# databendlabs/databend

Hardware: AMD Instinct MI355X
Metric: rows/s TPC-H Q1 hash-agg (higher is better)
Workload: dtype i64/i128 decimal

## Files before the change

### databend_amd/csrc/k_fagg.hip

```cpp
#include "fagg_device.h"
#include "runtime.h"

#include <dirent.h>
#include <dlfcn.h>
#include <errno.h>
#include <sys/stat.h>
#include <fcntl.h>
#include <signal.h>
#include <spawn.h>
#include <sys/wait.h>
#include <unistd.h>

#include <atomic>
#include <chrono>
#include <deque>
#include <map>
#include <mutex>
#include <string>

#include <stdlib.h>
#include <string.h>
#include <time.h>

using namespace dbhip;
// ... 495 lines not shown
    if (keys[k].type != L.key_type[k]) { set_error("dbhip_groupby_add_block_program: key %d has type %d, table expects %d", k, keys[k].type, L.key_type[k]); return DBHIP_ERR_INVALID; }
    if (keys[k].validity && !L.key_nullable[k]) { set_error("dbhip_groupby_add_block_program: key %d carries validity but was declared NOT NULL", k); return DBHIP_ERR_INVALID; }
    GbCol& c = A.key[k];
    c.data = keys[k].data; c.validity = keys[k].validity; c.voff = keys[k].validity_offset; c.buffers = keys[k].buffers;
    c.type = keys[k].type; c.is_scalar = keys[k].is_scalar;
    A.key_type[k] = L.key_type[k]; A.key_off[k] = L.key_off[k]; A.key_words[k] = L.key_words[k];
    A.key_has_valid[k] = keys[k].validity != nullptr;
  }
  *out_general = general; *out_nwords = nwords; *out_may_raise = may_raise;
  return DBHIP_OK;
}


static int32_t fa_launch(const FaArgs& A, int slots, bool general, int nwords, int grid, size_t lds, hipStream_t s) {
  bool jit_pending = false;
  hipFunction_t jf = jit_kernel(A, slots, general, nwords, (t_jit_only && !t_jit_may_compile) ? JIT_LOOKUP : JIT_BACKGROUND, &jit_pending);
  if (!jf && t_jit_only) {
    t_jit_pending = jit_pending;
    if (jit_pending) ++g_fa_pending_refusals;
    set_error("dbhip_fagg: the specialised kernel of this shape is %s", jit_pending ? "being compiled in the background" : "not available");
    return DBHIP_ERR_UNSUPPORTED;
  }
  if (jf) {
    size_t asz = sizeof(A);
    void* extra[] = {HIP_LAUNCH_PARAM_BUFFER_POINTER, (void*)&A, HIP_LAUNCH_PARAM_BUFFER_SIZE, &asz, HIP_LAUNCH_PARAM_END};
    DBHIP_CHECK(hipModuleLaunchKernel(jf, grid, 1, 1, 256, 1, 1, 0, s, nullptr, extra));
    ++g_fa_jit_launches;
    return DBHIP_OK;
  }
  ++g_fa_interp_launches;
#define FA_LAUNCH(SL, GEN)                                                                                     \
  do {                                                                                                         \
    if (nwords <= 4) hipLaunchKernelGGL((fagg_kernel<SL, GEN, 4>), dim3(grid), dim3(256), lds, s, A);           \
    else hipLaunchKernelGGL((fagg_kernel<SL, GEN, FA_MAXW>), dim3(grid), dim3(256), lds, s, A);                 \
  } while (0)
  bool has_div = false;
  for (int i = 0; i < A.P.n_ins; ++i) has_div |= A.P.ins[i].op == EX_DEC && dec_op_needs_division(A.P.dec[A.P.ins[i].dec_idx]);
  if (has_div && slots == 4) hipLaunchKernelGGL((fagg_kernel<4, true, FA_MAXW, true>), dim3(grid), dim3(256), lds, s, A);
  else if (has_div) hipLaunchKernelGGL((fagg_kernel<8, true, FA_MAXW, true>), dim3(grid), dim3(256), lds, s, A);
  else if (slots == 4 && !general) FA_LAUNCH(4, false);
  else if (slots == 4) FA_LAUNCH(4, true);
  else if (!general) FA_LAUNCH(8, false);
  else FA_LAUNCH(8, true);
#undef FA_LAUNCH
  return DBHIP_OK;
}

namespace {
constexpr int FA_PIPE_WINDOW = 2048;
constexpr int FA_PIPE_BATCH = 512;
constexpr size_t FA_PIPE_COPY_BYTES = 16384;
constexpr size_t FA_PIPE_TABLE_BYTES = 65536;
constexpr int FA_PIPE_RING = 8;
constexpr int64_t FA_PIPE_BIG = 8 << 20;
constexpr int64_t FA_PIPE_BATCH_ROWS = 32 << 20;
struct FaShape { FaArgs A; bool general; int nwords; size_t lds; std::string sig; };
struct FaPending { int shape; FaBlock b; };
struct FaMerge { uint64_t seq; int64_t rows_ub; int64_t blocks; };
struct FaPipe {
  bool on = false, bound = false, slots8 = false;
  bool given_up = false;
  hipStream_t stream = nullptr;
  uint64_t* rows = nullptr;
  int64_t cap_rows = 0;
  uint64_t* ctrl = nullptr;
  uint64_t* status_host = nullptr;
  uint64_t* status_dev = nullptr;
  int64_t rows_ub = 0, window_blocks = 0;
  uint64_t seq = 0;
  std::deque<FaMerge> merges;
  int64_t count_seen = 0;
  std::deque<FaPending> retained;
  int64_t retained_base = 0, submitted = 0;
  std::vector<FaPending> batch;
  int64_t batch_rows = 0;
  std::vector<FaShape> shapes;
  uint64_t* tab_host[FA_PIPE_RING] = {};
  uint64_t* tab_dev[FA_PIPE_RING] = {};
  hipEvent_t tab_ev[FA_PIPE_RING] = {};
  bool tab_used[FA_PIPE_RING] = {};
  int tab_next = 0;
};

__global__ void fa_pipe_seal_kernel(uint64_t* ctrl) {
  if (ctrl[2]) ctrl[1] |= 4;
}
__global__ void fa_pipe_commit_kernel(uint64_t* ctrl, const uint64_t* gctrl, uint64_t* status, uint64_t seq, uint64_t blocks) {
  if (gctrl[1]) ctrl[1] |= 8;
  const bool dirty = (ctrl[1] & 15) != 0;
  if (!dirty) ctrl[3] += blocks;
  ctrl[0] = 0;
  __hip_atomic_store(&status[1], gctrl[0] | (dirty ? (1ULL << 63) : 0ULL), __ATOMIC_RELAXED, __HIP_MEMORY_SCOPE_SYSTEM);
  __hip_atomic_store(&status[0], seq, __ATOMIC_RELEASE, __HIP_MEMORY_SCOPE_SYSTEM);
}

void fa_pipe_poll(FaPipe* pp) {
  uint64_t seq0, cnt, seq1;
  do {
    seq0 = __atomic_load_n(&pp->status_host[0], __ATOMIC_ACQUIRE);
    cnt = __atomic_load_n(&pp->status_host[1], __ATOMIC_ACQUIRE);
    seq1 = __atomic_load_n(&pp->status_host[0], __ATOMIC_ACQUIRE);
  } while (seq0 != seq1);
  const bool dirty = (cnt >> 63) != 0;
  while (!pp->merges.empty() && pp->merges.front().seq <= seq0) {
    if (!dirty) {
      int64_t drop = pp->merges.front().blocks;
      while (drop-- > 0 && !pp->retained.empty()) { pp->retained.pop_front(); ++pp->retained_base; }
    }
    pp->merges.pop_front();
    pp->count_seen = (int64_t)(cnt & ~(1ULL << 63));
  }
}

int32_t fa_pipe_queue_merge(dbhip_groupby* g, FaPipe* pp) {
  if (pp->window_blocks == 0) return DBHIP_OK;
  hipStream_t s = pp->stream;
  fa_pipe_poll(pp);
  int64_t ub = pp->count_seen + pp->rows_ub;
  for (const FaMerge& m : pp->merges) ub += m.rows_ub;
  if (ub * 135 > dbhip_groupby_capacity_internal(g) * 100) {
    const int32_t rc = dbhip_groupby_ensure_room_internal(g, pp->rows_ub, s);
    if (rc) return rc;
    fa_pipe_poll(pp);
    pp->merges.clear();
    pp->count_seen = dbhip_groupby_count_internal(g);
  }
  hipLaunchKernelGGL(fa_pipe_seal_kernel, dim3(1), dim3(1), 0, s, pp->ctrl);
  int32_t rc = dbhip_groupby_merge_rows_deferred_internal(g, pp->rows, pp->rows_ub, &pp->ctrl[0], &pp->ctrl[1], s);
  if (rc) return rc;
  ++pp->seq;
  hipLaunchKernelGGL(fa_pipe_commit_kernel, dim3(1), dim3(1), 0, s, pp->ctrl, dbhip_groupby_ctrl_internal(g), pp->status_dev, pp->seq,
                     (uint64_t)pp->window_blocks);
  DBHIP_LAUNCH_CHECK();
  pp->merges.push_back({pp->seq, pp->rows_ub, pp->window_blocks});
  pp->rows_ub = 0;
  pp->window_blocks = 0;
  return DBHIP_OK;
}

void fa_pipe_args(const FaPipe* pp, const FaPending& P, FaArgs& A) {
  A = pp->shapes[(size_t)P.shape].A;
  for (int c = 0; c < EX_MAX_INPUTS; ++c) { A.P.in_data[c] = P.b.in_data[c]; A.P.in_valid[c] = P.b.in_valid[c]; A.P.in_voff[c] = P.b.in_voff[c]; }
  for (int k = 0; k < FA_KW; ++k) { A.key[k].data = P.b.key_data[k]; A.key[k].validity = P.b.key_valid[k]; A.key[k].voff = P.b.key_voff[k]; }
  A.filter_bits = P.b.filter_bits; A.filter_off = P.b.filter_off; A.n = P.b.n;
}
int32_t fa_pipe_submit(dbhip_groupby* g, FaPipe* pp, const FaPending& P, hipStream_t s) {
  const FaShape& S = pp->shapes[(size_t)P.shape];
  FaArgs A;
  fa_pipe_args(pp, P, A);
  const int64_t nchunks = ceil_div(A.n, 64 * FA_ROWS);
  const int grid = (int)(ceil_div(nchunks, 4) < 512 ? ceil_div(nchunks, 4) : 512);
  const int64_t n_max = (int64_t)grid * FA_MAX_SLOTS;
  if (n_max > pp->cap_rows) { set_error("dbhip_groupby_add_block_program: grid too large for the pipeline's row buffer"); return DBHIP_ERR_INVALID; }
  if (pp->rows_ub + n_max > pp->cap_rows || pp->window_blocks >= FA_PIPE_WINDOW) {
    const int32_t rc = fa_pipe_queue_merge(g, pp);
    if (rc) return rc;
  }
  A.ctrl = pp->ctrl;
  A.partial_rows = pp->rows;
  A.P.err_words = nullptr;
  A.P.err_count = (unsigned long long*)&pp->ctrl[2];
  const int32_t rc = fa_launch(A, (pp->slots8 || pp->count_seen > 4) ? 8 : 4, S.general, S.nwords, grid, S.lds, s);
  if (rc) return rc;
  DBHIP_LAUNCH_CHECK();
  pp->rows_ub += n_max;
  ++pp->window_blocks;
  ++pp->submitted;
  pp->retained.push_back(P);
  return DBHIP_OK;
}

void fa_pack_block(const FaArgs& M, const FaBlock& b, uint64_t* w) {
  w[0] = (uint64_t)b.n;
  for (int ci = 0; ci < M.P.n_inputs; ++ci) {
    const int o = fa_blk_in_off(M, ci);
    w[o] = (uint64_t)b.in_data[ci];
    if (M.P.in_has_valid[ci]) { w[o + 1] = (uint64_t)b.in_valid[ci]; w[o + 2] = (uint64_t)b.in_voff[ci]; }
  }
  for (int q = 0; q < M.nkeys; ++q) {
    const int o = fa_blk_key_off(M, q);
    w[o] = (uint64_t)b.key_data[q];
    if (M.key_has_valid[q]) { w[o + 1] = (uint64_t)b.key_valid[q]; w[o + 2] = (uint64_t)b.key_voff[q]; }
  }
  if (M.has_filter) { const int o = fa_blk_filter_off(M); w[o] = (uint64_t)b.filter_bits; w[o + 1] = (uint64_t)b.filter_off; }
}

int32_t fa_pipe_flush_batch(dbhip_groupby* g, FaPipe* pp) {
  if (pp->batch.empty()) return DBHIP_OK;
  std::vector<FaPending> blocks;
  blocks.swap(pp->batch);
  pp->batch_rows = 0;
  hipStream_t s = pp->stream;
  const int nb = (int)blocks.size();
  const int slots = (pp->slots8 || pp->count_seen > 4) ? 8 : 4;
  const FaShape& S = pp->shapes[(size_t)blocks[0].shape];
  hipFunction_t jf = nb > 1 ? jit_kernel(S.A, slots, S.general, S.nwords, JIT_BACKGROUND, nullptr, true) : nullptr;
  if (!jf) {
    for (const FaPending& P : blocks) { const int32_t rc = fa_pipe_submit(g, pp, P, s); if (rc) return rc; }
    return DBHIP_OK;
  }
  const int64_t rpw = 64 * (int64_t)jit_rows(S.A);
  int64_t max_chunks = 1;
  for (const FaPending& P : blocks) { const int64_t c = ceil_div(P.b.n, rpw); max_chunks = c > max_chunks ? c : max_chunks; }
  int wpb = (int)(ceil_div(max_chunks, 4) < 512 / nb ? ceil_div(max_chunks, 4) : 512 / nb);
  if (wpb < 1) wpb = 1;
  const int grid = wpb * nb;
  const int64_t n_max = (int64_t)grid * FA_MAX_SLOTS;
  if (pp->rows_ub + n_max > pp->cap_rows || pp->window_blocks >= FA_PIPE_WINDOW) {
    const int32_t rc = fa_pipe_queue_merge(g, pp);
    if (rc) return rc;
  }
  const int slot = pp->tab_next;
  pp->tab_next = (pp->tab_next + 1) % FA_PIPE_RING;
  if (pp->tab_used[slot]) DBHIP_CHECK(hipEventSynchronize(pp->tab_ev[slot]));
  uint64_t* T = pp->tab_host[slot];
  const int bw = fa_blk_words(S.A);
  for (int i = 0; i < nb; ++i) fa_pack_block(S.A, blocks[i].b, T + (size_t)i * bw);
  for (size_t at = 0, all = (size_t)nb * bw * 8; at < all; at += FA_PIPE_COPY_BYTES)
    DBHIP_CHECK(hipMemcpyAsync((uint8_t*)pp->tab_dev[slot] + at, (const uint8_t*)T + at, all - at < FA_PIPE_COPY_BYTES ? all - at : FA_PIPE_COPY_BYTES,
                               hipMemcpyHostToDevice, s));
  DBHIP_CHECK(hipEventRecord(pp->tab_ev[slot], s));
  pp->tab_used[slot] = true;
  FaArgs A = S.A;
  A.ctrl = pp->ctrl; A.partial_rows = pp->rows;
  A.P.err_words = nullptr; A.P.err_count = (unsigned long long*)&pp->ctrl[2];
  A.blocks = pp->tab_dev[slot]; A.wgs_per_block = wpb;
  size_t asz = sizeof(A);
  void* extra[] = {HIP_LAUNCH_PARAM_BUFFER_POINTER, (void*)&A, HIP_LAUNCH_PARAM_BUFFER_SIZE, &asz, HIP_LAUNCH_PARAM_END};
  DBHIP_CHECK(hipModuleLaunchKernel(jf, grid, 1, 1, 256, 1, 1, 0, s, nullptr, extra));
  g_fa_jit_launches += 1;
  g_fa_multi_blocks += (uint64_t)nb;
  pp->rows_ub += n_max;
  pp->window_blocks += nb;
  pp->submitted += nb;
  for (const FaPending& P : blocks) pp->retained.push_back(P);
  return DBHIP_OK;
}

int32_t fa_pipe_enqueue(dbhip_groupby* g, FaPipe* pp, const FaPending& P, hipStream_t s) {
  if (P.b.n >= FA_PIPE_BIG || jit_mode() == 0) {
    const int32_t rc = fa_pipe_flush_batch(g, pp);
    return rc ? rc : fa_pipe_submit(g, pp, P, s);
  }
  if (!pp->batch.empty() && pp->batch[0].shape != P.shape) {
    const int32_t rc = fa_pipe_flush_batch(g, pp);
    if (rc) return rc;
  }
  pp->batch.push_back(P);
  pp->batch_rows += P.b.n;
  const int fit = (int)(FA_PIPE_TABLE_BYTES / ((size_t)fa_blk_words(pp->shapes[(size_t)P.shape].A) * 8));
  if ((int)pp->batch.size() >= (FA_PIPE_BATCH < fit ? FA_PIPE_BATCH : fit) || pp->batch_rows >= FA_PIPE_BATCH_ROWS) return fa_pipe_flush_batch(g, pp);
  return DBHIP_OK;
}

void fa_pipe_forget(FaPipe* pp) {
  pp->batch.clear(); pp->batch_rows = 0; pp->shapes.clear();
  pp->retained.clear(); pp->retained_base = 0; pp->submitted = 0; pp->merges.clear(); pp->rows_ub = 0; pp->window_blocks = 0;
}

int32_t fa_pipe_checkpoint(dbhip_groupby* g, FaPipe* pp, int64_t* out_committed, bool may_replay) {
  if (out_committed) *out_committed = 0;
  if (!pp->bound || (pp->submitted == 0 && pp->window_blocks == 0 && pp->batch.empty())) return DBHIP_OK;
  hipStream_t s = pp->stream;
  int32_t rc = fa_pipe_flush_batch(g, pp);
  if (rc) return rc;
  if ((rc = fa_pipe_queue_merge(g, pp))) return rc;
  uint64_t* h = pinned_words(2);
  if (!h) return DBHIP_ERR_HIP;
  DBHIP_CHECK(hipMemcpyAsync(h, pp->ctrl, 32, hipMemcpyDeviceToHost, s));
  DBHIP_CHECK(hipMemcpyAsync(h + 4, dbhip_groupby_ctrl_internal(g), 8, hipMemcpyDeviceToHost, s));
  DBHIP_CHECK(hipStreamSynchronize(s));
  const uint64_t flags = h[1], errs = h[2];
  const int64_t committed = (int64_t)h[3];
  dbhip_groupby_set_count_internal(g, (int64_t)h[4]);
  pp->merges.clear();
  pp->count_seen = (int64_t)h[4];
  if (!(flags & 15)) {
    fa_pipe_forget(pp);
    DBHIP_CHECK(hipMemsetAsync(pp->ctrl, 0, 64, s));
    if (out_committed) *out_committed = committed;
    return DBHIP_OK;
  }
  if ((flags & 15) == 1 && !pp->slots8 && may_replay) {
    pp->slots8 = true;
    std::deque<FaPending> again;
    const int64_t skip = committed - pp->retained_base;
    for (int64_t i = skip < 0 ? 0 : skip; i < (int64_t)pp->retained.size(); ++i) again.push_back(pp->retained[(size_t)i]);
    DBHIP_CHECK(hipMemsetAsync(pp->ctrl, 0, 24, s));
    pp->retained.clear(); pp->retained_base = committed; pp->submitted = committed; pp->rows_ub = 0; pp->window_blocks = 0;
    for (const FaPending& P : again)
      if ((rc = fa_pipe_enqueue(g, pp, P, s))) return rc;
    return fa_pipe_checkpoint(g, pp, out_committed, false);
  }
  const int64_t submitted = pp->submitted;
  fa_pipe_forget(pp);
  DBHIP_CHECK(hipMemsetAsync(pp->ctrl, 0, 64, s));
  if (out_committed) *out_committed = committed;
  if (flags & 2) {
    set_error("dbhip_groupby_checkpoint: a group key string is longer than 12 bytes; pipelined blocks [%lld, %lld) were not merged",
              (long long)committed, (long long)submitted);
    return DBHIP_ERR_UNSUPPORTED;
  }
  if (flags & 4) {
    set_error("dbhip_groupby_checkpoint: %llu row error(s) in the fused maps (Decimal overflow / divided by zero); pipelined blocks [%lld, %lld) were "
              "not merged: evaluate their maps with dbhip_expr_eval to get the rows", (unsigned long long)errs, (long long)committed, (long long)submitted);
    return DBHIP_ERR_ROW_ERRORS;
  }
  pp->given_up = true;
  set_error("dbhip_groupby_checkpoint: more than %d distinct groups inside one workgroup%s; pipelined blocks [%lld, %lld) were not merged: use the "
            "operator-at-a-time path for them", FA_MAX_SLOTS, (flags & 8) ? " (and the table filled during a merge)" : "", (long long)committed,
            (long long)submitted);
  return DBHIP_ERR_CAPACITY;
}
}

int32_t dbhip_fagg_pipe_drain_internal(dbhip_groupby* g, void* pipe, hipStream_t) {
  FaPipe* pp = (FaPipe*)pipe;
  if (!pp->bound || (pp->submitted == 0 && pp->window_blocks == 0 && pp->batch.empty())) return DBHIP_OK;
  int64_t committed = 0;
  return fa_pipe_checkpoint(g, pp, &committed, true);
}
int32_t dbhip_fagg_pipe_reset_internal(void* pipe, hipStream_t s) {
  FaPipe* pp = (FaPipe*)pipe;
  if (pp->bound) DBHIP_CHECK(hipStreamSynchronize(pp->stream));
  fa_pipe_forget(pp);
  pp->count_seen = 0; pp->slots8 = false; pp->bound = false; pp->given_up = false;
  DBHIP_CHECK(hipMemsetAsync(pp->ctrl, 0, 64, s));
  DBHIP_CHECK(hipStreamSynchronize(s));
  return DBHIP_OK;
}
void dbhip_fagg_pipe_destroy_internal(void* pipe) {
  FaPipe* pp = (FaPipe*)pipe;
  if (!pp) return;
  if (pp->rows) (void)dbhip_free(pp->rows);
  if (pp->ctrl) (void)hipFree(pp->ctrl);
  if (pp->status_host) (void)hipHostFree(pp->status_host);
  for (int i = 0; i < FA_PIPE_RING; ++i) {
    if (pp->tab_host[i]) (void)hipHostFree(pp->tab_host[i]);
    if (pp->tab_dev[i]) (void)hipFree(pp->tab_dev[i]);
    if (pp->tab_ev[i]) (void)hipEventDestroy(pp->tab_ev[i]);
  }
  delete pp;
}


extern "C" {

int32_t dbhip_groupby_add_block_program(dbhip_groupby* g, const dbhip_col* keys, const dbhip_agg_program* prog, int64_t n,
                                        const uint8_t* filter_bitmap, int64_t filter_bit_offset, void* stream) {
  DBHIP_REQUIRE(g && keys && prog && prog->arg_regs, "dbhip_groupby_add_block_program: NULL argument");
  const GbLayout& L = *dbhip_groupby_layout_internal(g);
  if (!dbhip_fagg_layout_ok_internal(L)) {
    set_error("dbhip_groupby_add_block_program: layout outside the fused kernel (<= %d key words, <= %d aggregates, <= %d state words)", FA_KW, FA_MAXA, FA_MAXW);
    return DBHIP_ERR_UNSUPPORTED;
  }
  if (n == 0) return DBHIP_OK;
  hipStream_t s = resolve_stream(stream);
  if (FaPipe* pp = (FaPipe*)*dbhip_groupby_pipe_slot_internal(g); pp && pp->on && !t_prepare_only && !t_jit_only) {
    if (pp->bound && pp->stream != s) {
      set_error("dbhip_groupby_add_block_program: a pipelined table takes its blocks on ONE stream (checkpoint before changing it)");
      return DBHIP_ERR_INVALID;
    }
    DBHIP_REQUIRE(prog->n_inputs >= 0 && prog->n_inputs <= EX_MAX_INPUTS && (prog->inputs || prog->n_inputs == 0), "expression program: 0..8 input columns");
    DBHIP_REQUIRE(prog->n_ins >= 0 && prog->n_ins <= 2 * EX_MAX_INS && (prog->prog || prog->n_ins == 0), "expression program: too many instructions");
    static thread_local std::string sig;
    sig.clear();
    auto put = [&](const void* p, size_t nb) { sig.append((const char*)p, nb); };
    put(&prog->n_ins, 4); put(&prog->n_inputs, 4); put(&prog->filter_reg, 4);
    if (prog->n_ins) put(prog->prog, (size_t)prog->n_ins * sizeof(dbhip_expr_ins));
    for (int c = 0; c < prog->n_inputs; ++c) {
      const dbhip_col& col = prog->inputs[c];
      DBHIP_REQUIRE(col.data, "expression program: NULL input column");
      const int32_t t[3] = {col.type, col.is_scalar, (int32_t)(col.validity != nullptr) | ((int32_t)col.precision << 8) | ((int32_t)col.scale << 16)};
      put(t, sizeof(t));
    }
    for (int k = 0; k < L.nkeys; ++k) {
      const int32_t t[3] = {keys[k].type, keys[k].is_scalar, (int32_t)(keys[k].validity != nullptr)};
      put(t, sizeof(t));
    }
    put(prog->arg_regs, (size_t)L.naggs * 4);
    const char hf = filter_bitmap != nullptr;
    put(&hf, 1);
    int sh = -1;
    for (int i = (int)pp->shapes.size() - 1; i >= 0 && sh < 0; --i)
      if (pp->shapes[(size_t)i].sig == sig) sh = i;
    if (sh < 0) {
      FaShape S;
      FaArgs A;
      memset(&A, 0, sizeof(A));
      bool may_raise = false;
      const int32_t rc = fa_build_args(L, keys, prog, A, &S.general, &S.nwords, &may_raise);
      if (rc) return rc;
      A.has_filter = filter_bitmap != nullptr;
      S.lds = (size_t)(A.P.n_slots > 6 ? A.P.n_slots : 6) * FA_ROWS * 256 * 8;
      if (S.lds > 60 * 1024) {
        set_error("dbhip_groupby_add_block_program: %d live LDS slots exceed the register file; split the expression", A.P.n_slots);
        return DBHIP_ERR_UNSUPPORTED;
      }
      fa_shape(A, S.A);
      S.sig = sig;
      pp->shapes.push_back(std::move(S));
      sh = (int)pp->shapes.size() - 1;
    }
    FaPending P;
    memset(&P.b, 0, sizeof(P.b));
    P.shape = sh;
    for (int c = 0; c < prog->n_inputs; ++c) {
      P.b.in_data[c] = prog->inputs[c].data; P.b.in_valid[c] = prog->inputs[c].validity; P.b.in_voff[c] = prog->inputs[c].validity_offset;
    }
    for (int k = 0; k < L.nkeys; ++k) { P.b.key_data[k] = keys[k].data; P.b.key_valid[k] = keys[k].validity; P.b.key_voff[k] = keys[k].validity_offset; }
    P.b.filter_bits = filter_bitmap; P.b.filter_off = filter_bit_offset; P.b.n = n;
    pp->bound = true; pp->stream = s;
    return fa_pipe_enqueue(g, pp, P, s);
  }
  FaArgs A;
  memset(&A, 0, sizeof(A));
  bool general = false, may_raise = false;
  int nwords = 0;
  int32_t rc = fa_build_args(L, keys, prog, A, &general, &nwords, &may_raise);
  if (rc) return rc;
  A.filter_bits = filter_bitmap; A.filter_off = filter_bit_offset; A.n = n;
  A.has_filter = filter_bitmap != nullptr;
  const size_t lds = (size_t)(A.P.n_slots > 6 ? A.P.n_slots : 6) * FA_ROWS * 256 * 8;
  if (lds > 60 * 1024) {
    set_error("dbhip_groupby_add_block_program: %d live LDS slots exceed the register file; split the expression", A.P.n_slots);
    return DBHIP_ERR_UNSUPPORTED;
  }
  const int64_t nchunks = ceil_div(n, 64 * FA_ROWS);
  const int grid = (int)(ceil_div(nchunks, 4) < 512 ? ceil_div(nchunks, 4) : 512);
  if (FaPipe* pp = (FaPipe*)*dbhip_groupby_pipe_slot_internal(g); pp && !t_prepare_only) {
    int64_t committed = 0;
    if ((rc = fa_pipe_checkpoint(g, pp, &committed, true))) return rc;
  }
  const size_t rows_bytes = (size_t)grid * FA_MAX_SLOTS * L.W * 8;
  uint8_t* ws = (uint8_t*)scratch(rows_bytes + 64, 6, s);
  if (!ws) return DBHIP_ERR_HIP;
  uint64_t* ctrl = (uint64_t*)ws;
  A.ctrl = ctrl;
  A.partial_rows = (uint64_t*)(ws + 64);
  A.P.err_words = nullptr;
  A.P.err_count = (unsigned long long*)&ctrl[2];
  uint64_t* host_ctrl = pinned_words(1);
  if (!host_ctrl) return DBHIP_ERR_HIP;
  host_ctrl[0] = host_ctrl[1] = host_ctrl[2] = 0;
  const int64_t n_max = (int64_t)grid * FA_MAX_SLOTS;
  const bool chained = (dbhip_groupby_count_internal(g) + n_max) * 135 <= dbhip_groupby_capacity_internal(g) * 100;
  if ((rc = dbhip_groupby_reserve_merge_internal(g, n_max))) return rc;
  if (t_prepare_only) {
    (void)jit_kernel(A, dbhip_groupby_count_internal(g) > 4 ? 8 : 4, general, nwords, JIT_COMPILE);
    if (FaPipe* pq = (FaPipe*)*dbhip_groupby_pipe_slot_internal(g); pq && pq->on)
      (void)jit_kernel(A, dbhip_groupby_count_internal(g) > 4 ? 8 : 4, general, nwords, JIT_COMPILE, nullptr, true);
    return DBHIP_OK;
  }
  for (int variant = dbhip_groupby_count_internal(g) > 4 ? 1 : 0; variant < 2; ++variant) {
    DBHIP_CHECK(hipMemsetAsync(ctrl, 0, 64, s));
    kernel_timer_start(s);
    if ((rc = fa_launch(A, variant == 0 ? 4 : 8, general, nwords, grid, lds, s))) return rc;
    kernel_timer_stop(s);
    DBHIP_LAUNCH_CHECK();
    DBHIP_CHECK(hipMemcpyAsync(host_ctrl, ctrl, 24, hipMemcpyDeviceToHost, s));
    if (chained && !may_raise) {
      rc = dbhip_groupby_merge_rows_dev_internal(g, A.partial_rows, n_max, &ctrl[0], &ctrl[1], s);
      if (rc) return rc;
      if (!(host_ctrl[1] & 3)) return DBHIP_OK;
    } else {
      DBHIP_CHECK(hipStreamSynchronize(s));
    }
    if (!(host_ctrl[1] & 1)) break;
  }
  if (host_ctrl[1] & 2) {
    set_error("dbhip_groupby_add_block_program: a group key string is longer than 12 bytes");
    return DBHIP_ERR_UNSUPPORTED;
  }
  if (host_ctrl[1] & 1) {
    set_error("dbhip_groupby_add_block_program: more than %d distinct groups inside one workgroup; use the operator-at-a-time path", FA_MAX_SLOTS);
    return DBHIP_ERR_CAPACITY;
  }
  if (host_ctrl[2]) {
    set_error("dbhip_groupby_add_block_program: %llu row error(s) in the fused maps (Decimal overflow / divided by zero); "
              "evaluate the maps with dbhip_expr_eval to get the rows", (unsigned long long)host_ctrl[2]);
    return DBHIP_ERR_ROW_ERRORS;
  }
  return dbhip_groupby_merge_rows_internal(g, A.partial_rows, (int64_t)host_ctrl[0], s);
}

int32_t dbhip_groupby_set_pipelined(dbhip_groupby* g, int32_t on, void* stream) {
  DBHIP_REQUIRE(g, "dbhip_groupby_set_pipelined: NULL argument");
  void** slot = dbhip_groupby_pipe_slot_internal(g);
  FaPipe* pp = (FaPipe*)*slot;
  if (!on) {
    if (!pp) return DBHIP_OK;
    int64_t committed = 0;
    const int32_t rc = fa_pipe_checkpoint(g, pp, &committed, true);
    pp->on = false; pp->bound = false;
    return rc;
  }
  const GbLayout& L = *dbhip_groupby_layout_internal(g);
  if (!dbhip_fagg_layout_ok_internal(L)) {
    set_error("dbhip_groupby_set_pipelined: layout outside the fused kernel (<= %d key words, <= %d aggregates, <= %d state words)", FA_KW, FA_MAXA, FA_MAXW);
    return DBHIP_ERR_UNSUPPORTED;
  }
  if (pp) { pp->on = true; return DBHIP_OK; }
  pp = new (std::nothrow) FaPipe();
  DBHIP_REQUIRE(pp, "dbhip_groupby_set_pipelined: out of host memory");
  hipStream_t s = resolve_stream(stream);
  pp->cap_rows = 65536;
  int32_t rc = dbhip_alloc((size_t)pp->cap_rows * L.W * 8, (void**)&pp->rows);
  hipError_t e = rc == DBHIP_OK ? hipMalloc((void**)&pp->ctrl, 64) : hipSuccess;
  if (rc == DBHIP_OK && e == hipSuccess) e = hipHostMalloc((void**)&pp->status_host, 64, hipHostMallocMapped);
  if (rc == DBHIP_OK && e == hipSuccess) e = hipHostGetDevicePointer((void**)&pp->status_dev, pp->status_host, 0);
  if (rc == DBHIP_OK && e == hipSuccess) { memset(pp->status_host, 0, 64); e = hipMemsetAsync(pp->ctrl, 0, 64, s); }
  if (rc == DBHIP_OK && e == hipSuccess) e = hipStreamSynchronize(s);
  for (int i = 0; i < FA_PIPE_RING && rc == DBHIP_OK && e == hipSuccess; ++i) {
    e = hipHostMalloc((void**)&pp->tab_host[i], FA_PIPE_TABLE_BYTES, hipHostMallocDefault);
    if (e == hipSuccess) e = hipMalloc((void**)&pp->tab_dev[i], FA_PIPE_TABLE_BYTES);
    if (e == hipSuccess) e = hipEventCreateWithFlags(&pp->tab_ev[i], hipEventDisableTiming);
  }
  if (rc == DBHIP_OK && e == hipSuccess) rc = dbhip_groupby_reserve_merge_internal(g, pp->cap_rows);
  if (rc != DBHIP_OK || e != hipSuccess) {
    dbhip_fagg_pipe_destroy_internal(pp);
    return rc != DBHIP_OK ? rc : hip_fail(e, "dbhip_groupby_set_pipelined");
  }
  pp->count_seen = dbhip_groupby_count_internal(g);
  pp->on = true;
  *slot = pp;
  return DBHIP_OK;
}

int32_t dbhip_groupby_checkpoint(dbhip_groupby* g, int64_t* out_blocks_committed_host, void* stream) {
  DBHIP_REQUIRE(g, "dbhip_groupby_checkpoint: NULL argument");
  if (out_blocks_committed_host) *out_blocks_committed_host = 0;
  FaPipe* pp = (FaPipe*)*dbhip_groupby_pipe_slot_internal(g);
  if (!pp) return DBHIP_OK;
  if (pp->bound && stream && pp->stream != resolve_stream(stream)) {
    set_error("dbhip_groupby_checkpoint: the table's blocks were queued on another stream");
    return DBHIP_ERR_INVALID;
  }
  const int32_t rc = fa_pipe_checkpoint(g, pp, out_blocks_committed_host, true);
  pp->bound = false;
  return rc;
}

int32_t dbhip_groupby_prepare_program(dbhip_groupby* g, const dbhip_col* keys, const dbhip_agg_program* prog) {
  t_prepare_only = true;
  const int32_t rc = dbhip_groupby_add_block_program(g, keys, prog, 1, nullptr, 0, nullptr);
  t_prepare_only = false;
  return rc;
}

}

static bool fa_offset_col(const GbCol& c, int64_t row0, dbhip_col* out) {
  memset(out, 0, sizeof(*out));
  out->type = c.type; out->is_scalar = c.is_scalar; out->buffers = c.buffers; out->validity = c.validity;
  out->validity_offset = c.voff + (c.is_scalar ? 0 : row0);
  if (c.is_scalar || row0 == 0) { out->data = c.data; return true; }
  if (c.type == DBHIP_T_BOOL) {
    if (row0 & 7) return false;
    out->data = (const uint8_t*)c.data + (row0 >> 3);
    return true;
  }
  const int es = type_size(c.type);
  if (es == 0) return false;
  out->data = (const uint8_t*)c.data + (size_t)row0 * es;
  return true;
}

int32_t dbhip_fagg_add_columns_internal(dbhip_groupby* g, const GbCols& C, int64_t row0, int64_t n, bool may_compile, hipStream_t s) {
  const GbLayout& L = *dbhip_groupby_layout_internal(g);
  if (!dbhip_fagg_layout_ok_internal(L)) return DBHIP_ERR_UNSUPPORTED;
  dbhip_col keys[FA_KW], inputs[EX_MAX_INPUTS];
  int32_t arg_regs[FA_MAXA];
  int n_inputs = 0;
  for (int k = 0; k < L.nkeys; ++k)
    if (!fa_offset_col(C.key[k], row0, &keys[k])) return DBHIP_ERR_UNSUPPORTED;
  bool any_arg = false;
  for (int a = 0; a < L.naggs; ++a) {
    arg_regs[a] = DBHIP_ARG_NONE;
    if (C.arg[a].data == nullptr) {
      if (L.agg_kind[a] != DBHIP_AGG_COUNT) return DBHIP_ERR_UNSUPPORTED;
      continue;
    }
    if (!fa_arg_type_ok(C.arg[a].type)) return DBHIP_ERR_UNSUPPORTED;
    int found = -1;
    dbhip_col col;
    if (!fa_offset_col(C.arg[a], row0, &col)) return DBHIP_ERR_UNSUPPORTED;
    for (int c = 0; c < n_inputs && found < 0; ++c)
      if (inputs[c].data == col.data && inputs[c].type == col.type && inputs[c].validity == col.validity &&
          inputs[c].validity_offset == col.validity_offset && inputs[c].is_scalar == col.is_scalar) found = c;
    if (found < 0) {
      if (n_inputs >= EX_MAX_INPUTS) return DBHIP_ERR_UNSUPPORTED;
      if (col.type == DBHIP_T_DEC128) { int wide = 0; for (int c = 0; c < n_inputs; ++c) wide += inputs[c].type == DBHIP_T_DEC128; if (wide >= 2) return DBHIP_ERR_UNSUPPORTED; }
      inputs[n_inputs] = col;
// ... 98 lines not shown
```

### databend_amd/host/block_sweep.cpp

```cpp
#include <stdint.h>
#include <stdio.h>
#include <stdlib.h>
#include <string.h>

#include <algorithm>
#include <atomic>
#include <chrono>
#include <string>
#include <thread>
#include <vector>

#include "../../include/dbhip.h"

#define CK(x)                                                                                   \
  do {                                                                                          \
    int32_t _rc = (x);                                                                          \
    if (_rc != DBHIP_OK) { fprintf(stderr, "%s:%d: %s -> %d: %s\n", __FILE__, __LINE__, #x, _rc, dbhip_last_error()); exit(2); } \
  } while (0)

static double now_s() { return std::chrono::duration<double>(std::chrono::steady_clock::now().time_since_epoch()).count(); }
static uint64_t mix(uint64_t x) { x += 0x9e3779b97f4a7c15ULL; x = (x ^ (x >> 30)) * 0xbf58476d1ce4e5b9ULL; x = (x ^ (x >> 27)) * 0x94d049bb133111ebULL; return x ^ (x >> 31); }

struct Lineitem {
  int64_t n = 0;
// ... 197 lines not shown
  dbhip_groupby* fin = tables[0];
  for (int t = 1; t < T; ++t) {
    int64_t n = 0, rb = 0, m = 0;
    CK(dbhip_groupby_num_groups(tables[t], &n, nullptr)); CK(dbhip_groupby_row_bytes(tables[t], &rb));
    void* d = dalloc((size_t)(n > 0 ? n : 1) * rb);
    CK(dbhip_groupby_flush_serialized(tables[t], d, n, &m, nullptr));
    CK(dbhip_groupby_merge_serialized(fin, d, m, nullptr));
    CK(dbhip_stream_sync(nullptr));
    CK(dbhip_free(d));
  }
  const Q1Result got = q1_result(fin);
  *ok = got.groups == expect.groups && got.words == expect.words;
  *calls_out = 0;
  for (int t = 0; t < T; ++t) *calls_out += calls[t];
  { double tot = 0; for (int t = 0; t < T; ++t) tot += in_call[t]; g_host_us = *calls_out ? tot / (double)*calls_out * 1e6 : 0; }
  for (int t = 0; t < T; ++t) { CK(dbhip_groupby_destroy(tables[t])); CK(dbhip_stream_destroy(streams[t])); }
  for (auto& S : staging) { dbhip_free(S.qty); dbhip_free(S.price); dbhip_free(S.disc); dbhip_free(S.tax); dbhip_free(S.ship); dbhip_free(S.rf); dbhip_free(S.ls); }
  return secs;
}

template <class F>
static double run_blocks(int64_t total, int64_t B, int T, F fn, int64_t* calls_out) {
  const int64_t nblocks = (total + B - 1) / B;
  std::vector<void*> streams(T);
  for (int t = 0; t < T; ++t) CK(dbhip_stream_create(&streams[t]));
  std::atomic<int> ready{0};
  std::atomic<bool> go{false};
  std::vector<double> t_end(T, 0.0);
  std::vector<std::thread> th;
  for (int t = 0; t < T; ++t) th.emplace_back([&, t] {
    ++ready;
    while (!go.load(std::memory_order_acquire)) {}
    for (int64_t b = t; b < nblocks; b += T) {
      const int64_t row0 = b * B, n = row0 + B <= total ? B : total - row0;
      fn(t, streams[t], row0, n);
    }
    CK(dbhip_stream_sync(streams[t]));
    t_end[t] = now_s();
  });
  while (ready.load() < T) {}
  const double t0 = now_s();
  go.store(true, std::memory_order_release);
  for (auto& x : th) x.join();
  double secs = 0;
  for (int t = 0; t < T; ++t) secs = t_end[t] - t0 > secs ? t_end[t] - t0 : secs;
  for (int t = 0; t < T; ++t) CK(dbhip_stream_destroy(streams[t]));
  *calls_out = nblocks;
  return secs;
}

int main(int argc, char** argv) {
  int64_t N = 64LL << 20;
  const char* out = nullptr;
  bool quick = false, only_q1 = false;
  for (int i = 1; i < argc; ++i) {
    if (!strcmp(argv[i], "--rows") && i + 1 < argc) N = atoll(argv[++i]);
    else if (!strcmp(argv[i], "--out") && i + 1 < argc) out = argv[++i];
    else if (!strcmp(argv[i], "--quick")) quick = true;
    else if (!strcmp(argv[i], "--only-q1")) only_q1 = true;
  }
  CK(dbhip_init(0));
  fprintf(stderr, "generating %lld lineitem rows ...\n", (long long)N);
  Lineitem li = gen_lineitem(N);

  Q1Result expect;
  {
    dbhip_groupby* g; CK(dbhip_q1_create_groupby(&g));
    Q1Program P; P.build(li, 0);
    CK(dbhip_groupby_prepare_program(g, P.keys, &P.ap));
    CK(dbhip_groupby_add_block_program(g, P.keys, &P.ap, N, nullptr, 0, nullptr));
    expect = q1_result(g);
    CK(dbhip_groupby_destroy(g));
    fprintf(stderr, "whole-table result: %llu groups\n", (unsigned long long)expect.groups);
  }
  std::vector<int64_t> sizes = {65536, 262144, 1 << 20, 16 << 20, N};
  std::vector<int> threads = {1, 8};
  if (quick) { sizes = {65536, 1 << 20}; }
  for (int rep = 0; rep < 2; ++rep) {
    if (rep == 1) g_lines.clear();
    for (int64_t B : sizes)
      for (int T : threads) {
        if (B >= N && T > 1) continue;
        for (Q1Mode mode : {Q1_SYNC, Q1_PIPE}) {
          bool ok = false; int64_t calls = 0;
          const double secs = run_q1(li, B, T, mode, 0, expect, &ok, &calls);
          Line l{mode == Q1_SYNC ? "q1_sync" : "q1_pipelined", B, T, secs, N, calls, ok, ""};
          l.host_us = g_host_us;
          report(l);
        }
      }
    if (!only_q1) for (int T : threads)
      for (int64_t S : {(int64_t)1 << 20, (int64_t)4 << 20})
        for (Q1Mode mode : {Q1_SQUASH, Q1_SQUASH_PIPE}) {
          bool ok = false; int64_t calls = 0;
          const double secs = run_q1(li, 65536, T, mode, S, expect, &ok, &calls);
          report({std::string(mode == Q1_SQUASH ? "q1_squash_" : "q1_squashpipe_") + (S == (1 << 20) ? "1Mi" : "4Mi"), 65536, T, secs, N, calls, ok, "device-to-device concat of 7 columns, then the call"});
        }
  }

  {
    auto make_table = [&](dbhip_groupby** g) {
      int32_t kt[1] = {DBHIP_T_I64}; uint8_t kn[1] = {0};
      dbhip_agg_desc ad[2]; memset(ad, 0, sizeof(ad));
      ad[0].kind = DBHIP_AGG_SUM; ad[0].arg_type = DBHIP_T_I64; ad[1].kind = DBHIP_AGG_COUNT;
      CK(dbhip_groupby_create(kt, kn, 1, ad, 2, 1024, g));
    };
    auto run_plain = [&](int64_t B, int T, bool pipelined, const Q1Result* expect, Q1Result* out_res, int64_t* calls_out) -> double {
      const int64_t nblocks = (li.n + B - 1) / B;
      std::vector<dbhip_groupby*> tables(T); std::vector<void*> streams(T);
      for (int t = 0; t < T; ++t) { make_table(&tables[t]); CK(dbhip_stream_create(&streams[t])); if (pipelined) CK(dbhip_groupby_set_pipelined(tables[t], 1, streams[t])); }
      static bool warmed = false;
      for (int t = 0; t < 1 && !warmed; ++t) {
        dbhip_col k = col(DBHIP_T_I64, li.k4), a[2]; a[0] = col(DBHIP_T_I64, li.price); memset(&a[1], 0, sizeof(a[1]));
        for (int w = 0; w < 40; ++w) { CK(dbhip_groupby_add_block(tables[t], &k, a, 65536, streams[t])); int64_t c; CK(dbhip_groupby_checkpoint(tables[t], &c, streams[t])); CK(dbhip_stream_sync(streams[t])); uint64_t st[3]; dbhip_fagg_stats(st); if (st[0] > 0 && w > 2) break; std::this_thread::sleep_for(std::chrono::milliseconds(100)); }
        for (int w = 0; w < 40 && pipelined; ++w) {
          uint64_t s0[3], s1[3]; dbhip_fagg_stats(s0);
          for (int q = 0; q < 2; ++q) CK(dbhip_groupby_add_block(tables[t], &k, a, 65536, streams[t]));
          int64_t c; CK(dbhip_groupby_checkpoint(tables[t], &c, streams[t]));
          dbhip_fagg_stats(s1);
          if (s1[0] - s0[0] == 1) break;
          std::this_thread::sleep_for(std::chrono::milliseconds(100));
        }
        CK(dbhip_groupby_reset(tables[t], streams[t]));
        warmed = pipelined;
      }
      std::atomic<int> ready{0}; std::atomic<bool> go{false};
      std::vector<double> t_end(T, 0.0);
      std::vector<std::thread> th;
      for (int t = 0; t < T; ++t) th.emplace_back([&, t] {
        ++ready;
// ... 110 lines not shown
```

Baseline: 94.48 billion.

## Run pipelined fused-agg launches on two side-stream lanes and cache last shape

Large blocks and JIT batch launches in the pipelined group-by path are now issued round-robin onto two extra non-blocking streams. Each lane waits on an event from the main stream and is joined back before the next merge, so consecutive aggregation kernels can overlap. Shape lookup first compares the new program signature against the last used shape in place, avoiding building a signature string per block. The change also adds abandon/cleanup handling and per-process lane limits. The risk is extra event and stream overhead, and possible contention on the shared partial-row buffer.

```diff
diff --git a/databend_amd/csrc/k_fagg.hip b/databend_amd/csrc/k_fagg.hip
--- a/databend_amd/csrc/k_fagg.hip
+++ b/databend_amd/csrc/k_fagg.hip
@@ -571,6 +571,10 @@
 constexpr size_t FA_PIPE_COPY_BYTES = 16384;
 constexpr size_t FA_PIPE_TABLE_BYTES = 65536;
 constexpr int FA_PIPE_RING = 8;
+constexpr int FA_PIPE_LANES = 2;
+#ifndef FA_PIPE_LANE_TABLES
+#define FA_PIPE_LANE_TABLES 64
+#endif
 constexpr int64_t FA_PIPE_BIG = 8 << 20;
 constexpr int64_t FA_PIPE_BATCH_ROWS = 32 << 20;
 struct FaShape { FaArgs A; bool general; int nwords; size_t lds; std::string sig; };
@@ -599,7 +603,45 @@
   hipEvent_t tab_ev[FA_PIPE_RING] = {};
   bool tab_used[FA_PIPE_RING] = {};
   int tab_next = 0;
+  int last_shape = -1;
+  bool lanes = false;
+  hipStream_t lane[FA_PIPE_LANES] = {};
+  hipEvent_t lane_in[FA_PIPE_LANES] = {};
+  hipEvent_t lane_done[FA_PIPE_LANES] = {};
+  bool lane_busy[FA_PIPE_LANES] = {};
+  int lane_next = 0;
 };
+std::atomic<int> g_fa_lane_tables{0};
+
+int32_t fa_lanes_join(FaPipe* pp) {
+  for (int l = 0; l < FA_PIPE_LANES; ++l)
+    if (pp->lane_busy[l]) {
+      DBHIP_CHECK(hipStreamWaitEvent(pp->stream, pp->lane_done[l], 0));
+      pp->lane_busy[l] = false;
+    }
+  return DBHIP_OK;
+}
+void fa_lanes_sync(FaPipe* pp) {
+  for (int l = 0; l < FA_PIPE_LANES; ++l)
+    if (pp->lane[l]) { (void)hipStreamSynchronize(pp->lane[l]); pp->lane_busy[l] = false; }
+  if (pp->bound) (void)hipStreamSynchronize(pp->stream);
+}
+int32_t fa_lane_begin(FaPipe* pp, hipStream_t* s, int* lane) {
+  *s = pp->stream; *lane = -1;
+  if (!pp->lanes) return DBHIP_OK;
+  const int l = pp->lane_next;
+  pp->lane_next = (l + 1) % FA_PIPE_LANES;
+  DBHIP_CHECK(hipEventRecord(pp->lane_in[l], pp->stream));
+  DBHIP_CHECK(hipStreamWaitEvent(pp->lane[l], pp->lane_in[l], 0));
+  *s = pp->lane[l]; *lane = l;
+  return DBHIP_OK;
+}
+int32_t fa_lane_end(FaPipe* pp, int lane) {
+  if (lane < 0) return DBHIP_OK;
+  pp->lane_busy[lane] = true;
+  DBHIP_CHECK(hipEventRecord(pp->lane_done[lane], pp->lane[lane]));
+  return DBHIP_OK;
+}
 
 __global__ void fa_pipe_seal_kernel(uint64_t* ctrl) {
   if (ctrl[2]) ctrl[1] |= 4;
@@ -632,8 +674,12 @@
 }
 
 int32_t fa_pipe_queue_merge(dbhip_groupby* g, FaPipe* pp) {
+  hipStream_t s = pp->stream;
+  {
+    const int32_t rc = fa_lanes_join(pp);
+    if (rc) return rc;
+  }
   if (pp->window_blocks == 0) return DBHIP_OK;
-  hipStream_t s = pp->stream;
   fa_pipe_poll(pp);
   int64_t ub = pp->count_seen + pp->rows_ub;
   for (const FaMerge& m : pp->merges) ub += m.rows_ub;
@@ -663,7 +709,7 @@
   for (int k = 0; k < FA_KW; ++k) { A.key[k].data = P.b.key_data[k]; A.key[k].validity = P.b.key_valid[k]; A.key[k].voff = P.b.key_voff[k]; }
   A.filter_bits = P.b.filter_bits; A.filter_off = P.b.filter_off; A.n = P.b.n;
 }
-int32_t fa_pipe_submit(dbhip_groupby* g, FaPipe* pp, const FaPending& P, hipStream_t s) {
+int32_t fa_pipe_submit(dbhip_groupby* g, FaPipe* pp, const FaPending& P) {
   const FaShape& S = pp->shapes[(size_t)P.shape];
   FaArgs A;
   fa_pipe_args(pp, P, A);
@@ -679,8 +725,12 @@
   A.partial_rows = pp->rows;
   A.P.err_words = nullptr;
   A.P.err_count = (unsigned long long*)&pp->ctrl[2];
-  const int32_t rc = fa_launch(A, (pp->slots8 || pp->count_seen > 4) ? 8 : 4, S.general, S.nwords, grid, S.lds, s);
+  hipStream_t s = pp->stream;
+  int lane = -1;
+  if (P.b.n >= FA_PIPE_BIG) { const int32_t rc = fa_lane_begin(pp, &s, &lane); if (rc) return rc; }
+  int32_t rc = fa_launch(A, (pp->slots8 || pp->count_seen > 4) ? 8 : 4, S.general, S.nwords, grid, S.lds, s);
   if (rc) return rc;
+  if ((rc = fa_lane_end(pp, lane))) return rc;
   DBHIP_LAUNCH_CHECK();
   pp->rows_ub += n_max;
   ++pp->window_blocks;
@@ -709,13 +759,12 @@
   std::vector<FaPending> blocks;
   blocks.swap(pp->batch);
   pp->batch_rows = 0;
-  hipStream_t s = pp->stream;
   const int nb = (int)blocks.size();
   const int slots = (pp->slots8 || pp->count_seen > 4) ? 8 : 4;
   const FaShape& S = pp->shapes[(size_t)blocks[0].shape];
   hipFunction_t jf = nb > 1 ? jit_kernel(S.A, slots, S.general, S.nwords, JIT_BACKGROUND, nullptr, true) : nullptr;
   if (!jf) {
-    for (const FaPending& P : blocks) { const int32_t rc = fa_pipe_submit(g, pp, P, s); if (rc) return rc; }
+    for (const FaPending& P : blocks) { const int32_t rc = fa_pipe_submit(g, pp, P); if (rc) return rc; }
     return DBHIP_OK;
   }
   const int64_t rpw = 64 * (int64_t)jit_rows(S.A);
@@ -729,6 +778,9 @@
     const int32_t rc = fa_pipe_queue_merge(g, pp);
     if (rc) return rc;
   }
+  hipStream_t s;
+  int lane;
+  { const int32_t rc = fa_lane_begin(pp, &s, &lane); if (rc) return rc; }
   const int slot = pp->tab_next;
   pp->tab_next = (pp->tab_next + 1) % FA_PIPE_RING;
   if (pp->tab_used[slot]) DBHIP_CHECK(hipEventSynchronize(pp->tab_ev[slot]));
@@ -747,6 +799,7 @@
   size_t asz = sizeof(A);
   void* extra[] = {HIP_LAUNCH_PARAM_BUFFER_POINTER, (void*)&A, HIP_LAUNCH_PARAM_BUFFER_SIZE, &asz, HIP_LAUNCH_PARAM_END};
   DBHIP_CHECK(hipModuleLaunchKernel(jf, grid, 1, 1, 256, 1, 1, 0, s, nullptr, extra));
+  { const int32_t rc = fa_lane_end(pp, lane); if (rc) return rc; }
   g_fa_jit_launches += 1;
   g_fa_multi_blocks += (uint64_t)nb;
   pp->rows_ub += n_max;
@@ -756,10 +809,10 @@
   return DBHIP_OK;
 }
 
-int32_t fa_pipe_enqueue(dbhip_groupby* g, FaPipe* pp, const FaPending& P, hipStream_t s) {
+int32_t fa_pipe_enqueue(dbhip_groupby* g, FaPipe* pp, const FaPending& P) {
   if (P.b.n >= FA_PIPE_BIG || jit_mode() == 0) {
     const int32_t rc = fa_pipe_flush_batch(g, pp);
-    return rc ? rc : fa_pipe_submit(g, pp, P, s);
+    return rc ? rc : fa_pipe_submit(g, pp, P);
   }
   if (!pp->batch.empty() && pp->batch[0].shape != P.shape) {
     const int32_t rc = fa_pipe_flush_batch(g, pp);
@@ -772,18 +825,54 @@
   return DBHIP_OK;
 }
 
+struct FaSigIns { int32_t op, dst, a, b, type, size; uint64_t imm; };
+static_assert(sizeof(FaSigIns) == 32, "FaSigIns is compared as bytes: no padding");
+template <class Put>
+void fa_signature(const GbLayout& L, const dbhip_col* keys, const dbhip_agg_program* prog, bool has_filter, Put&& put) {
+  const int32_t head[3] = {prog->n_ins, prog->n_inputs, prog->filter_reg};
+  put(head, sizeof(head));
+  for (int i = 0; i < prog->n_ins; ++i) {
+    const dbhip_expr_ins& I = prog->prog[i];
+    const FaSigIns f = {I.op, I.dst, I.a, I.b, I.type, (int32_t)I.precision | ((int32_t)I.scale << 8), I.imm};
+    put(&f, sizeof(f));
+  }
+  for (int c = 0; c < prog->n_inputs; ++c) {
+    const dbhip_col& col = prog->inputs[c];
+    const int32_t t[3] = {col.type, col.is_scalar, (int32_t)(col.validity != nullptr) | ((int32_t)col.precision << 8) | ((int32_t)col.scale << 16)};
+    put(t, sizeof(t));
+  }
+  for (int k = 0; k < L.nkeys; ++k) {
+    const int32_t t[3] = {keys[k].type, keys[k].is_scalar, (int32_t)(keys[k].validity != nullptr)};
+    put(t, sizeof(t));
+  }
+  put(prog->arg_regs, (size_t)L.naggs * 4);
+  const char hf = has_filter;
+  put(&hf, 1);
+}
+
 void fa_pipe_forget(FaPipe* pp) {
-  pp->batch.clear(); pp->batch_rows = 0; pp->shapes.clear();
+  pp->batch.clear(); pp->batch_rows = 0; pp->shapes.clear(); pp->last_shape = -1;
   pp->retained.clear(); pp->retained_base = 0; pp->submitted = 0; pp->merges.clear(); pp->rows_ub = 0; pp->window_blocks = 0;
+}
+int32_t fa_pipe_abandon(FaPipe* pp, int32_t rc) {
+  fa_lanes_sync(pp);
+  fa_pipe_forget(pp);
+  if (hipMemsetAsync(pp->ctrl, 0, 64, pp->stream) == hipSuccess) (void)hipStreamSynchronize(pp->stream);
+  pp->bound = false;
+  return rc;
 }
 
 int32_t fa_pipe_checkpoint(dbhip_groupby* g, FaPipe* pp, int64_t* out_committed, bool may_replay) {
   if (out_committed) *out_committed = 0;
-  if (!pp->bound || (pp->submitted == 0 && pp->window_blocks == 0 && pp->batch.empty())) return DBHIP_OK;
+  if (!pp->bound) return DBHIP_OK;
+  if (pp->submitted == 0 && pp->window_blocks == 0 && pp->batch.empty()) {
+    pp->bound = false;
+    return DBHIP_OK;
+  }
   hipStream_t s = pp->stream;
   int32_t rc = fa_pipe_flush_batch(g, pp);
-  if (rc) return rc;
-  if ((rc = fa_pipe_queue_merge(g, pp))) return rc;
+  if (rc) return fa_pipe_abandon(pp, rc);
+  if ((rc = fa_pipe_queue_merge(g, pp))) return fa_pipe_abandon(pp, rc);
   uint64_t* h = pinned_words(2);
   if (!h) return DBHIP_ERR_HIP;
   DBHIP_CHECK(hipMemcpyAsync(h, pp->ctrl, 32, hipMemcpyDeviceToHost, s));
@@ -796,6 +885,7 @@
   pp->count_seen = (int64_t)h[4];
   if (!(flags & 15)) {
     fa_pipe_forget(pp);
+    pp->bound = false;
     DBHIP_CHECK(hipMemsetAsync(pp->ctrl, 0, 64, s));
     if (out_committed) *out_committed = committed;
     return DBHIP_OK;
@@ -808,11 +898,12 @@
     DBHIP_CHECK(hipMemsetAsync(pp->ctrl, 0, 24, s));
     pp->retained.clear(); pp->retained_base = committed; pp->submitted = committed; pp->rows_ub = 0; pp->window_blocks = 0;
     for (const FaPending& P : again)
-      if ((rc = fa_pipe_enqueue(g, pp, P, s))) return rc;
+      if ((rc = fa_pipe_enqueue(g, pp, P))) return fa_pipe_abandon(pp, rc);
     return fa_pipe_checkpoint(g, pp, out_committed, false);
   }
   const int64_t submitted = pp->submitted;
   fa_pipe_forget(pp);
+  pp->bound = false;
   DBHIP_CHECK(hipMemsetAsync(pp->ctrl, 0, 64, s));
   if (out_committed) *out_committed = committed;
   if (flags & 2) {
@@ -841,7 +932,7 @@
 }
 int32_t dbhip_fagg_pipe_reset_internal(void* pipe, hipStream_t s) {
   FaPipe* pp = (FaPipe*)pipe;
-  if (pp->bound) DBHIP_CHECK(hipStreamSynchronize(pp->stream));
+  fa_lanes_sync(pp);
   fa_pipe_forget(pp);
   pp->count_seen = 0; pp->slots8 = false; pp->bound = false; pp->given_up = false;
   DBHIP_CHECK(hipMemsetAsync(pp->ctrl, 0, 64, s));
@@ -851,6 +942,13 @@
 void dbhip_fagg_pipe_destroy_internal(void* pipe) {
   FaPipe* pp = (FaPipe*)pipe;
   if (!pp) return;
+  fa_lanes_sync(pp);
+  for (int l = 0; l < FA_PIPE_LANES; ++l) {
+    if (pp->lane[l]) (void)hipStreamDestroy(pp->lane[l]);
+    if (pp->lane_in[l]) (void)hipEventDestroy(pp->lane_in[l]);
+    if (pp->lane_done[l]) (void)hipEventDestroy(pp->lane_done[l]);
+  }
+  if (pp->lanes) --g_fa_lane_tables;
   if (pp->rows) (void)dbhip_free(pp->rows);
   if (pp->ctrl) (void)hipFree(pp->ctrl);
   if (pp->status_host) (void)hipHostFree(pp->status_host);
@@ -882,27 +980,25 @@
     }
     DBHIP_REQUIRE(prog->n_inputs >= 0 && prog->n_inputs <= EX_MAX_INPUTS && (prog->inputs || prog->n_inputs == 0), "expression program: 0..8 input columns");
     DBHIP_REQUIRE(prog->n_ins >= 0 && prog->n_ins <= 2 * EX_MAX_INS && (prog->prog || prog->n_ins == 0), "expression program: too many instructions");
+    for (int c = 0; c < prog->n_inputs; ++c) DBHIP_REQUIRE(prog->inputs[c].data, "expression program: NULL input column");
+    int sh = -1;
+    if (pp->last_shape >= 0) {
+      const std::string& last = pp->shapes[(size_t)pp->last_shape].sig;
+      size_t at = 0;
+      bool same = true;
+      fa_signature(L, keys, prog, filter_bitmap != nullptr, [&](const void* p, size_t nb) {
+        same = same && at + nb <= last.size() && memcmp(last.data() + at, p, nb) == 0;
+        at += nb;
+      });
+      if (same && at == last.size()) sh = pp->last_shape;
+    }
     static thread_local std::string sig;
-    sig.clear();
-    auto put = [&](const void* p, size_t nb) { sig.append((const char*)p, nb); };
-    put(&prog->n_ins, 4); put(&prog->n_inputs, 4); put(&prog->filter_reg, 4);
-    if (prog->n_ins) put(prog->prog, (size_t)prog->n_ins * sizeof(dbhip_expr_ins));
-    for (int c = 0; c < prog->n_inputs; ++c) {
-      const dbhip_col& col = prog->inputs[c];
-      DBHIP_REQUIRE(col.data, "expression program: NULL input column");
-      const int32_t t[3] = {col.type, col.is_scalar, (int32_t)(col.validity != nullptr) | ((int32_t)col.precision << 8) | ((int32_t)col.scale << 16)};
-      put(t, sizeof(t));
-    }
-    for (int k = 0; k < L.nkeys; ++k) {
-      const int32_t t[3] = {keys[k].type, keys[k].is_scalar, (int32_t)(keys[k].validity != nullptr)};
-      put(t, sizeof(t));
-    }
-    put(prog->arg_regs, (size_t)L.naggs * 4);
-    const char hf = filter_bitmap != nullptr;
-    put(&hf, 1);
-    int sh = -1;
-    for (int i = (int)pp->shapes.size() - 1; i >= 0 && sh < 0; --i)
-      if (pp->shapes[(size_t)i].sig == sig) sh = i;
+    if (sh < 0) {
+      sig.clear();
+      fa_signature(L, keys, prog, filter_bitmap != nullptr, [&](const void* p, size_t nb) { sig.append((const char*)p, nb); });
+      for (int i = (int)pp->shapes.size() - 1; i >= 0 && sh < 0; --i)
+        if (pp->shapes[(size_t)i].sig == sig) sh = i;
+    }
     if (sh < 0) {
       FaShape S;
       FaArgs A;
@@ -921,6 +1017,7 @@
       pp->shapes.push_back(std::move(S));
       sh = (int)pp->shapes.size() - 1;
     }
+    pp->last_shape = sh;
     FaPending P;
     memset(&P.b, 0, sizeof(P.b));
     P.shape = sh;
@@ -930,7 +1027,7 @@
     for (int k = 0; k < L.nkeys; ++k) { P.b.key_data[k] = keys[k].data; P.b.key_valid[k] = keys[k].validity; P.b.key_voff[k] = keys[k].validity_offset; }
     P.b.filter_bits = filter_bitmap; P.b.filter_off = filter_bit_offset; P.b.n = n;
     pp->bound = true; pp->stream = s;
-    return fa_pipe_enqueue(g, pp, P, s);
+    return fa_pipe_enqueue(g, pp, P);
   }
   FaArgs A;
   memset(&A, 0, sizeof(A));
@@ -1011,7 +1108,7 @@
     if (!pp) return DBHIP_OK;
     int64_t committed = 0;
     const int32_t rc = fa_pipe_checkpoint(g, pp, &committed, true);
-    pp->on = false; pp->bound = false;
+    pp->on = false;
     return rc;
   }
   const GbLayout& L = *dbhip_groupby_layout_internal(g);
@@ -1035,6 +1132,14 @@
     if (e == hipSuccess) e = hipMalloc((void**)&pp->tab_dev[i], FA_PIPE_TABLE_BYTES);
     if (e == hipSuccess) e = hipEventCreateWithFlags(&pp->tab_ev[i], hipEventDisableTiming);
   }
+  if (rc == DBHIP_OK && e == hipSuccess) {
+    if (g_fa_lane_tables.fetch_add(1) < FA_PIPE_LANE_TABLES) pp->lanes = true; else --g_fa_lane_tables;
+  }
+  for (int l = 0; l < FA_PIPE_LANES && pp->lanes && e == hipSuccess; ++l) {
+    e = hipStreamCreateWithFlags(&pp->lane[l], hipStreamNonBlocking);
+    if (e == hipSuccess) e = hipEventCreateWithFlags(&pp->lane_in[l], hipEventDisableTiming);
+    if (e == hipSuccess) e = hipEventCreateWithFlags(&pp->lane_done[l], hipEventDisableTiming);
+  }
   if (rc == DBHIP_OK && e == hipSuccess) rc = dbhip_groupby_reserve_merge_internal(g, pp->cap_rows);
   if (rc != DBHIP_OK || e != hipSuccess) {
     dbhip_fagg_pipe_destroy_internal(pp);
@@ -1055,9 +1160,7 @@
     set_error("dbhip_groupby_checkpoint: the table's blocks were queued on another stream");
     return DBHIP_ERR_INVALID;
   }
-  const int32_t rc = fa_pipe_checkpoint(g, pp, out_blocks_committed_host, true);
-  pp->bound = false;
-  return rc;
+  return fa_pipe_checkpoint(g, pp, out_blocks_committed_host, true);
 }
 
 int32_t dbhip_groupby_prepare_program(dbhip_groupby* g, const dbhip_col* keys, const dbhip_agg_program* prog) {
diff --git a/databend_amd/host/block_sweep.cpp b/databend_amd/host/block_sweep.cpp
--- a/databend_amd/host/block_sweep.cpp
+++ b/databend_amd/host/block_sweep.cpp
@@ -273,12 +273,13 @@
 int main(int argc, char** argv) {
   int64_t N = 64LL << 20;
   const char* out = nullptr;
-  bool quick = false, only_q1 = false;
+  bool quick = false, only_q1 = false, one_thread = false;
   for (int i = 1; i < argc; ++i) {
     if (!strcmp(argv[i], "--rows") && i + 1 < argc) N = atoll(argv[++i]);
     else if (!strcmp(argv[i], "--out") && i + 1 < argc) out = argv[++i];
     else if (!strcmp(argv[i], "--quick")) quick = true;
     else if (!strcmp(argv[i], "--only-q1")) only_q1 = true;
+    else if (!strcmp(argv[i], "--one-thread")) one_thread = true;
   }
   CK(dbhip_init(0));
   fprintf(stderr, "generating %lld lineitem rows ...\n", (long long)N);
@@ -297,6 +298,7 @@
   std::vector<int64_t> sizes = {65536, 262144, 1 << 20, 16 << 20, N};
   std::vector<int> threads = {1, 8};
   if (quick) { sizes = {65536, 1 << 20}; }
+  if (one_thread) threads = {1};
   for (int rep = 0; rep < 2; ++rep) {
     if (rep == 1) g_lines.clear();
     for (int64_t B : sizes)
```

New measurement: 94.52 billion (median of 4 runs). Within noise of the previous version (+0.0%).
